# q8888620002/Group-Attribution-for-Diffusion-Models

Hardware: AMD Instinct MI355X
Metric: shapley_coalitions_per_hour (higher is better)
Workload: dtype f32; 1 GPU; CIFAR-20 DDPM sFT coalition (BASELINE configs[1]): gd_steps=1000 @B=128 + 10240 samples x 100 DDIM steps @B=32 (32 batches fused/launch), UNet2DModel widths [128, 256, 256, 256] 35.75M params fp32; step = 1/1000 coalition = 1 train step + 1 sampler step @B=1024, enqueued on 3 HIP streams (the train step belongs to a later coalition: independent work); coalitions_in_flight=3

## Files before the change

group-attribution-for-diffusion-models_amd/csrc/gemm_f32.hip:

```cpp
#include "gad_common.h"
#include "gemm_dev.h"

using namespace gadk;

namespace gadk {
void launch_wino4_fused(const DevArgs& w, int bm, hipStream_t st);
}

namespace {

template <int ROWS, int VEC>
struct LoadKCDense : KCSlots<ROWS> {
  using S = KCSlots<ROWS>;
  const float* base;
  long roff[S::NS];
  unsigned rowmask;
  int kend, k;
  bool kok;
  __device__ void init(const float* b, int ld, int row0, int nrows, int kend_) {
    base = b;
    kend = kend_;
    rowmask = 0;
#pragma unroll
    for (int i = 0; i < S::NS; ++i) {
// ... 2067 lines not shown

static int pick_vec(const gad_gemm_args* a) {
  int vec = 4;
  const int am = a->a_mode, bmode = a->b_mode;
  if (am == GAD_A_KC && (a->K % 4 != 0 || a->lda % 4 != 0)) vec = 1;
  if (am == GAD_A_MC && (a->M % 4 != 0 || a->lda % 4 != 0)) vec = 1;
  if (bmode == GAD_B_KC && (a->K % 4 != 0 || a->ldb % 4 != 0)) vec = 1;
  if (bmode == GAD_B_MC && (a->N % 4 != 0 || a->ldb % 4 != 0)) vec = 1;
  if ((am == GAD_A_CONV || am == GAD_A_CONVT || bmode == GAD_B_CONV) && (a->g.C % 4 != 0 || a->g.ldx % 4 != 0)) vec = 1;
  if (a->batch > 1 && (a->strideA0 % 4 != 0 || a->strideA1 % 4 != 0 || a->strideB0 % 4 != 0 || a->strideB1 % 4 != 0)) vec = 1;
  return vec;
}

enum : int32_t {
  HINT_128 = 1,
  HINT_64 = 2,
  HINT_128x64 = 3,
  HINT_WGRAD_96 = 4, HINT_WGRAD_64 = 5, HINT_WGRAD_32 = 6,
  HINT_WINO2 = 7,
  HINT_WINO4 = 8,
  HINT_WINO4_FUSED32 = 9,
  HINT_WINO4_THREE = 10,
  HINT_WINO4_FUSED64 = 11,
  HINT_SPLIT_M = 1000,
};

struct Plan {
  int bm, bn, tiles_m, tiles_n, splitk, ktiles_per_split;
  long nblocks;
};

static bool dense_128x64_ok(const gad_gemm_args* a) {
  const bool dense = (a->a_mode == GAD_A_KC || a->a_mode == GAD_A_MC) && (a->b_mode == GAD_B_KC || a->b_mode == GAD_B_MC) &&
                     !(a->a_mode == GAD_A_MC && a->b_mode == GAD_B_KC);
  return dense && !a->A2 && pick_vec(a) == 4 && !(a->operand_precision == 1);
}
static Plan make_plan(const gad_gemm_args* a) {
  const long batch = a->batch > 0 ? a->batch : 1;
  const int kt = (int)gad_ceil_div(a->K, BK) > 0 ? (int)gad_ceil_div(a->K, BK) : 1;
  static const int sks[] = {1, 2, 3, 4, 6, 8, 12, 16, 24, 32, 48, 64, 96, 128};
  double best = 1e30;
  Plan pl{};
  for (int bm = 128; bm >= 64; bm -= 64) {
    if (a->tile_hint == HINT_128 && bm != 128) continue;
    if (a->tile_hint == HINT_64 && bm != 64) continue;
    const bool bf = a->operand_precision == 1 && pick_vec(a) == 4;
// ... 350 lines not shown
  PatchPlan pp;
  if (use_patch_conv_f32(a, &pp)) {
    t_direct = (double)gad_ceil_div(pp.blocks, 512) * pp.chunks_per_split * 9.0 * (128.0 * pp.bn * 64.0) / 0.264e12;
    if (pp.splitk > 1) t_direct += 4e-6 + (double)a->M * a->N * 4.0 * (pp.splitk + 1) / 3.0e12;
  } else {
    t_direct = 2.0 * a->M * (double)a->N * a->K / 110e12;
  }
  const double tw = t2 < t4 ? t2 : t4;
  if (!(tw < 0.9 * t_direct)) return false;
  *wp = t2 < t4 ? p2 : p4;
  return true;
}

struct WinoWgradPlan {
  long T;
  int64_t wy_bytes, v_bytes, du_bytes, bytes;
};
static bool use_wino_wgrad(const gad_gemm_args* a, WinoWgradPlan* wq) {
  const gad_conv_geom& g = a->g;
  if (!(a->flags & GAD_GEMM_WINO_WGRAD) || (a->flags & (GAD_GEMM_NO_WINO | GAD_GEMM_NO_PATCH | GAD_GEMM_INTERNAL_WINO4))) return false;
  if (a->operand_precision != 0 || a->a_mode != GAD_A_MC || a->b_mode != GAD_B_CONV || a->A2 || a->A_k2 || a->batch > 1) return false;
  if (!same_3x3(g) || (g.Ho & 3) || (g.Wo & 3)) return false;
  if (g.C % 4 != 0 || g.ldx % 4 != 0 || a->M % 4 != 0 || a->lda % 4 != 0 || a->N != 9 * g.C || a->ldc % 4 != 0) return false;
  if ((a->tile_hint != 0 && a->tile_hint != HINT_WINO4) || a->splitk_hint > 0 || a->K % (g.Ho * g.Wo) != 0) return false;
  if (a->alpha != 1.f || a->bias || a->rowadd || a->residual) return false;
  if (!(gad_aligned16(a->A) && gad_aligned16(a->B) && gad_aligned16(a->C))) return false;
  wq->T = (long)a->K / 16;
  wq->wy_bytes = (int64_t)36 * wq->T * a->M * 4;
  wq->v_bytes = (int64_t)36 * wq->T * g.C * 4;
  wq->du_bytes = (int64_t)36 * a->M * g.C * 4;
  wq->bytes = wq->wy_bytes + wq->v_bytes + wq->du_bytes;
  if (a->tile_hint == HINT_WINO4) return true;
  const double dy_bytes = 4.0 * a->K * a->M, x_bytes = 4.0 * (double)(a->K / (g.Ho * g.Wo)) * g.H * g.W * g.C;
  const double t_w = (dy_bytes + x_bytes + (double)wq->wy_bytes + (double)wq->v_bytes) / 4.9e12 + 36.0 * wq->T * a->M * (double)g.C * 2.0 / 100e12 +
                     3.0 * (double)wq->du_bytes / 3.0e12 + 30e-6;
  const double t_direct = 2.0 * a->K * (double)a->M * a->N / 115e12;
  return t_w < 0.9 * t_direct;
}


static gad_gemm_args products36(const gad_gemm_args* a, const float* A, const float* B, float* C, int am, int bm, int M, int N, int K) {
  gad_gemm_args sub = *a;
  sub.A = A; sub.B = B; sub.C = C;
  sub.a_mode = am; sub.b_mode = bm;
  sub.M = M; sub.N = N; sub.K = K;
  sub.lda = am == GAD_A_MC ? M : K; sub.ldb = bm == GAD_B_MC ? N : K; sub.ldc = N;
  sub.batch = 36; sub.batch_inner = 1;
  sub.strideA0 = (int64_t)M * K; sub.strideB0 = (int64_t)N * K; sub.strideC0 = (int64_t)M * N;
  sub.strideA1 = sub.strideB1 = sub.strideC1 = 0;
  sub.tile_hint = 0; sub.splitk_hint = 0;
  sub.flags = GAD_GEMM_INTERNAL_WINO4;
  sub.B_wino = nullptr; sub.B_wino4 = nullptr; sub.wino_ws = nullptr; sub.wino_ws_bytes = 0;
  sub.A2 = nullptr;
  return sub;
}
// ... 257 lines not shown
  GAD_CHECK(a->wino_ws && a->wino_ws_bytes >= wq.bytes && gad_aligned16(a->wino_ws),
            "gad_gemm: Winograd weight-gradient workspace too small or misaligned (%lld < %lld)", (long long)a->wino_ws_bytes, (long long)wq.bytes);
  float* Wy = (float*)a->wino_ws;
  float* V = Wy + wq.wy_bytes / 4;
  float* dU = V + wq.v_bytes / 4;
  const bool have_v = (a->flags & GAD_GEMM_WINO_SKIP_INPUT) && a->B_wino4 != nullptr;
  if (have_v) {
    GAD_CHECK(gad_aligned16(a->B_wino4), "gad_gemm: the kept Winograd input image (B_wino4 of a weight-gradient launch) must be 16-byte aligned");
    V = const_cast<float*>(a->B_wino4);
  }
  WinoIn wy;
  wy.x = a->A; wy.V = Wy;
  wy.H = g.Ho; wy.W = g.Wo; wy.C = a->M; wy.ldx = a->lda; wy.up = 0;
  wy.TH = g.Ho / 4; wy.TW = g.Wo / 4; wy.T = wq.T;
  WinoIn wi;
  wi.x = a->B; wi.V = V;
  wi.H = g.H; wi.W = g.W; wi.C = g.C; wi.ldx = g.ldx; wi.up = g.upsample ? 1 : 0;
  wi.TH = wy.TH; wi.TW = wy.TW; wi.T = wq.T;
  const long iy = wq.T * (a->M / 4), ix = wq.T * (g.C / 4);
  GAD_CHECK(gad_ceil_div(iy, 256) < (1L << 31) && gad_ceil_div(ix, 256) < (1L << 31), "gad_gemm: Winograd transform grid too large");
  hipLaunchKernelGGL(wino4_dy_kernel, dim3((unsigned)gad_ceil_div(iy, 256)), dim3(256), 0, st, wy);
  if (!have_v) hipLaunchKernelGGL(wino4_input_kernel, dim3((unsigned)gad_ceil_div(ix, 256)), dim3(256), 0, st, wi);
  GAD_LAUNCH_CHECK("gad_gemm(winograd wgrad transforms)");
  const gad_gemm_args sub = wino_wgrad_products_args(a, wq, Wy, V, dU);
  if (const int rc = gad_gemm(&sub, stream)) return rc;
  const long items = (long)a->M * (g.C / 4);
  hipLaunchKernelGGL(wino4_dw_kernel, dim3((unsigned)gad_ceil_div(items, 256)), dim3(256), 0, st, dU, a->C, a->M, g.C, a->ldc);
  GAD_LAUNCH_CHECK("gad_gemm(winograd wgrad output transform)");
  return 0;
}

static int launch_wino(const Route& r, const DevArgs& d, void* stream) {
  const gad_gemm_args* a = &r.a;
  const WinoPlan& wp = r.wp;
  const gad_conv_geom& g = a->g;
  hipStream_t st = (hipStream_t)stream;
  GAD_CHECK(a->wino_ws && a->wino_ws_bytes >= wp.bytes && gad_aligned16(a->wino_ws) && gad_aligned16(wp.f == 2 ? a->B_wino : a->B_wino4),
            "gad_gemm: Winograd workspace too small or misaligned (%lld < %lld)", (long long)a->wino_ws_bytes, (long long)wp.bytes);
  WinoIn wi;
  wi.x = a->A; wi.V = (float*)a->wino_ws;
  wi.H = g.H; wi.W = g.W; wi.C = g.C; wi.ldx = g.ldx; wi.up = g.upsample ? 1 : 0;
  wi.TH = g.Ho / wp.f; wi.TW = g.Wo / wp.f; wi.T = wp.T;
  const long items = wp.T * (g.C / 4);
  GAD_CHECK(gad_ceil_div(items, 256) < (1L << 31), "gad_gemm: Winograd input transform grid too large");
  const bool only_input = (a->flags & GAD_GEMM_WINO_ONLY_INPUT) != 0, skip_input = (a->flags & GAD_GEMM_WINO_SKIP_INPUT) != 0;
  auto products = [&](const float* U) {
    DevArgs w = d;
    w.A = wi.V; w.B = U;
// ... 260 lines not shown
```

group-attribution-for-diffusion-models_amd/gad/_capi.py:

```python
import ctypes as C
import os

_HERE = os.path.dirname(os.path.abspath(__file__))
LIB_PATH = os.path.join(_HERE, "libgad_hip.so")


class GadError(RuntimeError):
    pass


class ConvGeom(C.Structure):
    _fields_ = [("H", C.c_int32), ("W", C.c_int32), ("C", C.c_int32), ("ldx", C.c_int32),
                ("Ho", C.c_int32), ("Wo", C.c_int32), ("KH", C.c_int32), ("KW", C.c_int32),
                ("stride", C.c_int32), ("pad_t", C.c_int32), ("pad_l", C.c_int32), ("upsample", C.c_int32)]


class GemmArgs(C.Structure):
    _fields_ = [("A", C.c_void_p), ("B", C.c_void_p), ("C", C.c_void_p),
                ("a_mode", C.c_int32), ("b_mode", C.c_int32),
                ("M", C.c_int32), ("N", C.c_int32), ("K", C.c_int32),
                ("lda", C.c_int32), ("ldb", C.c_int32), ("ldc", C.c_int32),
                ("batch", C.c_int32), ("batch_inner", C.c_int32),
                ("strideA0", C.c_int64), ("strideA1", C.c_int64), ("strideB0", C.c_int64),
                ("strideB1", C.c_int64), ("strideC0", C.c_int64), ("strideC1", C.c_int64),
# ... 49 lines not shown
                ("tile_hint", C.c_int32), ("splitk_hint", C.c_int32)]


class AdamArgs(C.Structure):
    _fields_ = [("p", C.c_void_p), ("g", C.c_void_p), ("m", C.c_void_p), ("v", C.c_void_p), ("ema", C.c_void_p),
                ("n", C.c_int64), ("sumsq", C.c_void_p), ("max_norm", C.c_float),
                ("lr", C.c_float), ("beta1", C.c_float), ("beta2", C.c_float), ("eps", C.c_float),
                ("weight_decay", C.c_float), ("adamw", C.c_int32), ("step", C.c_int32), ("ema_decay", C.c_float)]


class JLArgs(C.Structure):
    _fields_ = [("A", C.c_void_p), ("lda", C.c_int64), ("G", C.c_int32), ("P", C.c_int64), ("p0", C.c_int64),
                ("d", C.c_int32), ("seed", C.c_uint32), ("model_id", C.c_uint32), ("type", C.c_int32),
                ("accumulate", C.c_int32), ("out", C.c_void_p), ("workspace", C.c_void_p), ("workspace_bytes", C.c_int64)]


class HGemmSegArgs(C.Structure):
    _fields_ = [("A", C.c_void_p), ("B", C.c_void_p), ("C", C.c_void_p), ("ws", C.c_void_p), ("ws_bytes", C.c_int64),
                ("c_seg_stride", C.c_int64), ("M", C.c_int32), ("N", C.c_int32), ("L", C.c_int32), ("S", C.c_int32),
                ("lda", C.c_int32), ("ldb", C.c_int32), ("ldc", C.c_int32), ("alpha", C.c_float), ("accumulate", C.c_int32),
                ("splitk_hint", C.c_int32)]


JL_NORMAL, JL_RADEMACHER = 0, 1
POOL_MAX, POOL_AVG, POOL_AVG_VALID = 0, 1, 2
GELU_ERF, GELU_QUICK = 0, 1
SIM_X_F32, SIM_X_U8 = 0, 1

GEMM_NO_PATCH, GEMM_TAP_MAJOR_K, GEMM_SCALAR_EPILOGUE, GEMM_GENERAL_LOADERS, GN_TWO_PASS = 1, 2, 4, 8, 1
GEMM_NO_WINO = 16
GEMM_WINO_WGRAD = 32
GEMM_WINO_ONLY_INPUT, GEMM_WINO_SKIP_INPUT = 64, 128
A_KC, A_MC, A_CONV, A_CONVT = 0, 1, 2, 3
B_KC, B_MC, B_WDGRAD, B_CONV = 0, 1, 2, 3

_vp, _i32, _i64, _f32, _f64 = C.c_void_p, C.c_int32, C.c_int64, C.c_float, C.c_double

SIGNATURES = {
    "gad_version": (C.c_int, []),
    "gad_last_error": (C.c_char_p, []),
    "gad_gemm_workspace_bytes": (_i64, [C.POINTER(GemmArgs)]),
    "gad_gemm": (C.c_int, [C.POINTER(GemmArgs), _vp]),
    "gad_gemm_uses_bf16": (C.c_int, [C.POINTER(GemmArgs)]),
    "gad_gemm_kernel_id": (C.c_int, [C.POINTER(GemmArgs)]),
    "gad_gemm_wino_bytes": (_i64, [C.POINTER(GemmArgs)]),
    "gad_wino_weights": (C.c_int, [_vp, _vp, _vp, _i64, _vp]),
    "gad_wino4_weights": (C.c_int, [_vp, _vp, _vp, _i64, _vp]),
    "gad_groupnorm_one_pass": (C.c_int, [C.POINTER(GroupNormArgs)]),
    "gad_gemm_plan": (C.c_int, [C.POINTER(GemmArgs), C.POINTER(_i32), C.POINTER(_i32), C.POINTER(_i32)]),
    "gad_groupnorm_workspace_bytes": (_i64, [C.POINTER(GroupNormArgs)]),
    "gad_groupnorm_silu_fwd": (C.c_int, [C.POINTER(GroupNormArgs), _vp]),
    "gad_groupnorm_silu_bwd": (C.c_int, [C.POINTER(GroupNormArgs), _vp]),
    "gad_groupnorm_wino4_ok": (C.c_int, [C.POINTER(GroupNormArgs), C.c_int32]),
    "gad_groupnorm_silu_wino4": (C.c_int, [C.POINTER(GroupNormArgs), _vp, C.c_int32, _vp]),
    "gad_attention_supported": (C.c_int, [_i32]),
    "gad_attention_uses_bf16": (C.c_int, [C.POINTER(AttentionArgs), _i32]),
    "gad_attention_bwd_workspace_bytes": (_i64, [C.POINTER(AttentionArgs)]),
    "gad_attention_fwd": (C.c_int, [C.POINTER(AttentionArgs), _vp]),
    "gad_attention_bwd": (C.c_int, [C.POINTER(AttentionArgs), _vp]),
    "gad_attention_d512_supported": (C.c_int, [_i32]),
    "gad_attention_fwd_d512": (C.c_int, [C.POINTER(AttentionArgs), _vp]),
    "gad_attention_causal_supported": (C.c_int, [_i32, _i32]),
    "gad_attention_causal_fwd": (C.c_int, [C.POINTER(AttentionArgs), _vp]),
    "gad_softmax_fwd": (C.c_int, [_vp, _vp, _i64, _i32, _f32, _vp]),
    "gad_softmax_bwd": (C.c_int, [_vp, _vp, _vp, _i64, _i32, _f32, _vp]),
    "gad_layernorm_workspace_bytes": (_i64, [_i64, _i32]),
    "gad_layernorm_fwd": (C.c_int, [_vp, _vp, _vp, _vp, _vp, _vp, _i64, _i32, _f32, _vp]),
    "gad_layernorm_bwd": (C.c_int, [_vp, _vp, _vp, _vp, _vp, _vp, _vp, _vp, _i64, _i32, _vp, _i64, _vp]),
    "gad_geglu_fwd": (C.c_int, [_vp, _vp, _i64, _i32, _vp]),
    "gad_geglu_bwd": (C.c_int, [_vp, _vp, _vp, _i64, _i32, _vp]),
# ... 91 lines not shown
```

group-attribution-for-diffusion-models_amd/gad/ops.py:

```python
from __future__ import annotations

import ctypes as C
import math
from typing import Optional

import torch

from . import _capi
from ._capi import (A_CONV, A_CONVT, A_KC, A_MC, B_CONV, B_KC, B_MC, B_WDGRAD, AdamArgs, ConvGeom, GemmArgs,
                    GroupNormArgs, check)
from .shadows import (WEIGHT_EPOCH, Shadow, cached, in_flat_buffer as _in_flat_buffer, weight_key, written,
                      written_everywhere)

_WS = {}
WS_BYTES = 1 << 30


def _stream():
    return C.c_void_p(torch.cuda.current_stream().cuda_stream)


_raw_stream = getattr(torch._C, "_cuda_getCurrentRawStream", None)


# ... 201 lines not shown
                a.B_wino4 = wino_v.data_ptr()
                a.flags |= _capi.GEMM_WINO_SKIP_INPUT
        else:
            a.flags &= ~_capi.GEMM_WINO_WGRAD
    if wino_input is not None:
        if lib.gad_gemm_kernel_id(C.byref(a)) != 6 or not a.wino_ws:
            return False
        wino_input(V)
        a.flags |= _capi.GEMM_WINO_SKIP_INPUT
    if ROUTE_STATS is not None and (a.B_wino4 or a.flags & _capi.GEMM_WINO_WGRAD):
        key = (lib.gad_gemm_kernel_id(C.byref(a)), M, N, K, bool(a.flags & _capi.GEMM_WINO_SKIP_INPUT), torch.is_grad_enabled())
        ROUTE_STATS[key] = ROUTE_STATS.get(key, 0) + 1
    if SCRATCH_ALLOC is not None:
        need = lib.gad_gemm_workspace_bytes(C.byref(a))
        ws = _scratch("ws", need, A.device) if need else None
        a.ws, a.ws_bytes = (ws.data_ptr() if need else None), need
    if PROFILER is not None:
        PROFILER.gemm(lib, a, batch)
        return True
    check(lib.gad_gemm(C.byref(a), _stream()), "gad_gemm")
    return True


class GemmProfiler:
    NAMES = {(A_CONV, B_KC): "conv_fwd", (A_CONVT, B_WDGRAD): "conv_dgrad", (A_MC, B_CONV): "conv_wgrad",
             (A_KC, B_KC): "gemm_nt", (A_KC, B_MC): "gemm_nn", (A_MC, B_MC): "gemm_tn"}

    def __init__(self):
        self.records = []

    def gemm(self, lib, a, batch):
        tile, sk, vec = C.c_int32(), C.c_int32(), C.c_int32()
        check(lib.gad_gemm_plan(C.byref(a), C.byref(tile), C.byref(sk), C.byref(vec)), "gad_gemm_plan")
        kid = lib.gad_gemm_kernel_id(C.byref(a))
        s, e, mid = torch.cuda.Event(enable_timing=True), torch.cuda.Event(enable_timing=True), None
        s.record()
        if kid in (5, 6) and not (a.flags & _capi.GEMM_WINO_SKIP_INPUT):
            flags = a.flags
            mid = torch.cuda.Event(enable_timing=True)
            a.flags = flags | _capi.GEMM_WINO_ONLY_INPUT
            check(lib.gad_gemm(C.byref(a), _stream()), "gad_gemm")
            mid.record()
            a.flags = flags | _capi.GEMM_WINO_SKIP_INPUT
            check(lib.gad_gemm(C.byref(a), _stream()), "gad_gemm")
            a.flags = flags
        else:
            check(lib.gad_gemm(C.byref(a), _stream()), "gad_gemm")
        e.record()
        name = self.NAMES.get((a.a_mode, a.b_mode), "gemm") + ("", "_bf16", f"_patch_w{a.g.Wo}", f"_patch_bf16_w{a.g.Wo}", f"_fewout_valu_w{a.g.Wo}", "_wino", "_wino4", "_wino4")[kid]
        key = (name, tile.value, sk.value, vec.value)
        g = a.g
        if a.a_mode in (A_CONV, A_CONVT):
            a_elems = (a.M // max(1, g.Ho * g.Wo)) * g.H * g.W * g.C
        else:
            a_elems = a.M * a.K
        b_elems = (a.K // max(1, g.Ho * g.Wo)) * g.H * g.W * g.C if a.b_mode == B_CONV else a.N * a.K
        extra = a.M * a.N if a.residual else 0
        nbytes = 4.0 * max(1, batch) * (a_elems + b_elems + a.M * a.N + extra)
        flops = 2.0 * a.M * a.N * a.K * max(1, batch)
        executed = flops * ({5: 16.0 / 36.0, 6: 0.25, 7: 0.25}.get(kid, 1.0))
        stage = None
        if kid in (5, 6):
            npos, tpx = (16, 4) if kid == 5 else (36, 16)
            v_bytes = 4.0 * npos * (a.M // tpx) * g.C
            stage = (mid, 4.0 * a_elems + v_bytes if mid is not None else 0.0, v_bytes + 4.0 * (b_elems * npos / 9.0 + a.M * a.N + extra))
        self.records.append((key, flops, nbytes, s, e, executed, stage))

    def hgemm(self, lib, a, tn=False):
        s, e = torch.cuda.Event(enable_timing=True), torch.cuda.Event(enable_timing=True)
        if tn:
            s.record()
            check(lib.gad_hgemm_tn(C.byref(a), _stream()), "gad_hgemm_tn")
            e.record()
            nbytes = 2.0 * a.K * (a.M + a.N) + 4.0 * a.M * a.N
            flops = 2.0 * a.M * a.N * a.K
            self.records.append((("hgemm_tn_wgrad", 128, 0, 8), flops, nbytes, s, e, flops, None))
            return
        tile, sk = C.c_int32(), C.c_int32()
        check(lib.gad_hgemm_plan(C.byref(a), C.byref(tile), C.byref(sk)), "gad_hgemm_plan")
        s.record()
        check(lib.gad_hgemm(C.byref(a), _stream()), "gad_hgemm")
        e.record()
        if a.conv:
            name = f"hconv{a.KH}x{a.KW}" + ("_s2dgrad" if a.conv == 2 else "_s2" if a.stride == 2 else "_up" if a.upsample else "")
            a_elems = (a.M // max(1, a.Ho * a.Wo)) * a.H * a.W * a.Cin
        else:
            name = "hgemm_wgrad" if a.out_f32 else "hgemm_lora" if a.A2 else "hgemm"
            a_elems = a.M * a.K
        nbytes = 2.0 * (a_elems + a.N * a.K + (a.M * a.N if a.residual else 0)) + (4.0 if a.out_f32 else 2.0) * a.M * a.N
        flops = 2.0 * a.M * a.N * a.K
# ... 238 lines not shown
        return dxe
    g = ConvGeom(Ho, Wo, Cout, Cout, He, We, KH, KW, stride, pad[0], pad[2], 0)
    gemm_raw(dy, wk, dxe, A_CONVT, B_WDGRAD, Bn * He * We, Cin, KH * KW * Cout, 0, 0, Cin, geom=g,
             tile_hint=tile_hint, splitk_hint=splitk_hint)
    return _upsample2x_bwd(dxe, x_shape) if upsample else dxe


def _upsample2x_bwd(dxe, x_shape):
    Bn, H, W, Cin = x_shape
    dx = torch.empty((Bn, H, W, Cin), device=dxe.device, dtype=torch.float32)
    check(_capi.load().gad_upsample2x_bwd(dxe.data_ptr(), dx.data_ptr(), Bn, H, W, Cin, _stream()), "gad_upsample2x_bwd")
    return dx


def conv2d_wgrad_raw(dy, x, w_like, stride=1, pad=(1, 1, 1, 1), upsample=False, tile_hint=0, splitk_hint=0, out=None, wino_v=None):
    _req(dy, "conv dy")
    _req(x, "conv x")
    Bn, H, W, Cin = x.shape
    Cout, _, KH, KW = w_like.shape
    _, Ho, Wo, _ = dy.shape
    dwk = _out((Cout, KH, KW, Cin), dy.device) if out is None else weight_krsc(out)
    if (KH == 1 and KW == 1 and stride == 1 and tuple(pad) == (0, 0, 0, 0) and not upsample and Cin % 4 == 0 and Cout % 4 == 0
            and not KERNEL_FLAGS["gemm"] & _capi.GEMM_GENERAL_LOADERS):
        gemm_raw(dy, x, dwk, A_MC, B_MC, Cout, Cin, Bn * H * W, Cout, Cin, Cin, tile_hint=tile_hint, splitk_hint=splitk_hint)
        return dwk.permute(0, 3, 1, 2)
    g = ConvGeom(H, W, Cin, Cin, Ho, Wo, KH, KW, stride, pad[0], pad[2], int(upsample))
    wino = (KH == 3 and KW == 3 and stride == 1 and tuple(pad) == (1, 1, 1, 1) and tile_hint in (0, 8) and splitk_hint == 0
            and Ho % 4 == 0 and Wo % 4 == 0 and OPERAND_PRECISION[0] == 0 and not KERNEL_FLAGS.get("no_wino4")
            and not KERNEL_FLAGS["gemm"] & (_capi.GEMM_NO_WINO | _capi.GEMM_NO_PATCH | _capi.GEMM_SCALAR_EPILOGUE | _capi.GEMM_TAP_MAJOR_K
                                            | _capi.GEMM_GENERAL_LOADERS))
    gemm_raw(dy, x, dwk, A_MC, B_CONV, Cout, KH * KW * Cin, Bn * Ho * Wo, Cout, 0, KH * KW * Cin, geom=g,
             tile_hint=tile_hint, splitk_hint=splitk_hint, wino_wgrad=wino, wino_v=wino_v)
    return dwk.permute(0, 3, 1, 2)


def colsum_raw(dy2d: torch.Tensor, segments=1, out=None):
    lib = _capi.load()
    ws = workspace(dy2d.device)
    rows, N = dy2d.shape
    if out is None:
        out = torch.empty((segments, N), device=dy2d.device, dtype=torch.float32)
    check(lib.gad_colsum(dy2d.data_ptr(), out.data_ptr(), segments, rows // segments, N, ws.data_ptr(), ws.numel(),
                         _stream()), "gad_colsum")
    return out


def linear_fwd_raw(x2d, w, bias=None, residual=None, alpha=1.0, force_f32=False):
    M, K = x2d.shape
    N = w.shape[0]
    y = _out((M, N), x2d.device)
# ... 146 lines not shown

def layernorm_fwd_raw(x, gamma, beta, eps):
    C_ = x.shape[-1]
    rows = x.numel() // C_
    y = torch.empty_like(x)
    stats = torch.empty((2, rows), device=x.device, dtype=torch.float32)
    check(_capi.load().gad_layernorm_fwd(x.data_ptr(), y.data_ptr(), gamma.data_ptr(), beta.data_ptr(), stats[0].data_ptr(),
                                         stats[1].data_ptr(), rows, C_, eps, _stream()), "gad_layernorm_fwd")
    return y, stats[0], stats[1]


def linear_dgrad_raw(dy2d, w):
    M, N = dy2d.shape
    K = w.shape[1]
    dx = _out((M, K), dy2d.device)
    gemm_raw(dy2d, w, dx, A_KC, B_MC, M, K, N, N, K, K)
    return dx


def linear_wgrad_raw(dy2d, x2d, out=None):
    M, N = dy2d.shape
    K = x2d.shape[1]
    dw = _out((N, K), dy2d.device) if out is None else out
    gemm_raw(dy2d, x2d, dw, A_MC, B_MC, N, K, M, N, K, K)
    return dw


def _param_grad(param, compute):
    v, first = _sink(param)
    if v is None:
        return compute(None)
    if first:
        compute(v)
    else:
        v.add_(compute(None))
    return None


def _conv_backward(ctx, dy, x, x_shape, w, stride, pad, upsample, has, need):
    dy = dy.contiguous()
    dx = None
    if need[0]:
        if dgrad_as_forward(w, stride, pad):
            dx = conv2d_fwd_raw(dy, rotated_weight(w), None)
            if upsample:
                dx = _upsample2x_bwd(dx, x_shape)
        else:
# ... 829 lines not shown
```

include/gad.h:

```cpp
#ifndef GAD_H
#define GAD_H
#include <stdint.h>
#ifdef __cplusplus
extern "C" {
#endif

int gad_version(void);
const char* gad_last_error(void);

enum gad_a_mode {
  GAD_A_KC = 0,
  GAD_A_MC = 1,
  GAD_A_CONV = 2,
  GAD_A_CONVT = 3
};
enum gad_b_mode {
  GAD_B_KC = 0,
  GAD_B_MC = 1,
  GAD_B_WDGRAD = 2,
  GAD_B_CONV = 3
};

typedef struct gad_conv_geom {
  int32_t H, W, C;
// ... 37 lines not shown
  void* wino_ws;
  int64_t wino_ws_bytes;
  const float* B_wino4;
} gad_gemm_args;
enum gad_gemm_flags {
  GAD_GEMM_NO_WINO = 16,
  GAD_GEMM_WINO_WGRAD = 32,
  GAD_GEMM_NO_PATCH = 1,
  GAD_GEMM_TAP_MAJOR_K = 2,
  GAD_GEMM_SCALAR_EPILOGUE = 4,
  GAD_GEMM_GENERAL_LOADERS = 8,
  GAD_GEMM_WINO_ONLY_INPUT = 64,
  GAD_GEMM_WINO_SKIP_INPUT = 128
};

int64_t gad_gemm_workspace_bytes(const gad_gemm_args* a);
int gad_gemm_plan(const gad_gemm_args* a, int32_t* tile, int32_t* splitk, int32_t* vec);
int gad_gemm(const gad_gemm_args* a, void* stream);
int gad_gemm_uses_bf16(const gad_gemm_args* a);
int gad_gemm_kernel_id(const gad_gemm_args* a);
int64_t gad_gemm_wino_bytes(const gad_gemm_args* a);
int gad_wino_weights(const float* src, float* dst, const int64_t* table, int64_t n_tiles, void* stream);
int gad_wino4_weights(const float* src, float* dst, const int64_t* table, int64_t n_tiles, void* stream);

typedef struct gad_groupnorm_args {
  const float* x;
  float* y;
  const float* gamma;
  const float* beta;
  float* mean;
  float* rstd;
  const float* dy;
  float* dgamma;
  float* dbeta;
  int32_t B, HW, C, G;
  float eps;
  int32_t silu;
  void* ws;
  int64_t ws_bytes;
  const float* x2;
  int32_t C1;
  int32_t flags;
  const float* dx_add;
} gad_groupnorm_args;
enum gad_groupnorm_flags { GAD_GN_TWO_PASS = 1 };

// ... 225 lines not shown
```

Baseline: 45.81 coalitions/hour.

## Add dedicated TN split-K GEMM kernel for weight gradients and Winograd products

```diff
diff --git a/group-attribution-for-diffusion-models_amd/csrc/gemm_f32.hip b/group-attribution-for-diffusion-models_amd/csrc/gemm_f32.hip
--- a/group-attribution-for-diffusion-models_amd/csrc/gemm_f32.hip
+++ b/group-attribution-for-diffusion-models_amd/csrc/gemm_f32.hip
@@ -2113,6 +2113,7 @@
   HINT_WINO4_FUSED32 = 9,
   HINT_WINO4_THREE = 10,
   HINT_WINO4_FUSED64 = 11,
+  HINT_WINO4_TN = 12,
   HINT_SPLIT_M = 1000,
 };
 
@@ -2509,7 +2510,7 @@
   if (a->operand_precision != 0 || a->a_mode != GAD_A_MC || a->b_mode != GAD_B_CONV || a->A2 || a->A_k2 || a->batch > 1) return false;
   if (!same_3x3(g) || (g.Ho & 3) || (g.Wo & 3)) return false;
   if (g.C % 4 != 0 || g.ldx % 4 != 0 || a->M % 4 != 0 || a->lda % 4 != 0 || a->N != 9 * g.C || a->ldc % 4 != 0) return false;
-  if ((a->tile_hint != 0 && a->tile_hint != HINT_WINO4) || a->splitk_hint > 0 || a->K % (g.Ho * g.Wo) != 0) return false;
+  if ((a->tile_hint != 0 && a->tile_hint != HINT_WINO4 && a->tile_hint != HINT_WINO4_TN) || a->splitk_hint > 0 || a->K % (g.Ho * g.Wo) != 0) return false;
   if (a->alpha != 1.f || a->bias || a->rowadd || a->residual) return false;
   if (!(gad_aligned16(a->A) && gad_aligned16(a->B) && gad_aligned16(a->C))) return false;
   wq->T = (long)a->K / 16;
@@ -2517,7 +2518,7 @@
   wq->v_bytes = (int64_t)36 * wq->T * g.C * 4;
   wq->du_bytes = (int64_t)36 * a->M * g.C * 4;
   wq->bytes = wq->wy_bytes + wq->v_bytes + wq->du_bytes;
-  if (a->tile_hint == HINT_WINO4) return true;
+  if (a->tile_hint == HINT_WINO4 || a->tile_hint == HINT_WINO4_TN) return true;
   const double dy_bytes = 4.0 * a->K * a->M, x_bytes = 4.0 * (double)(a->K / (g.Ho * g.Wo)) * g.H * g.W * g.C;
   const double t_w = (dy_bytes + x_bytes + (double)wq->wy_bytes + (double)wq->v_bytes) / 4.9e12 + 36.0 * wq->T * a->M * (double)g.C * 2.0 / 100e12 +
                      3.0 * (double)wq->du_bytes / 3.0e12 + 30e-6;
@@ -2821,8 +2822,28 @@
   hipLaunchKernelGGL(wino4_dy_kernel, dim3((unsigned)gad_ceil_div(iy, 256)), dim3(256), 0, st, wy);
   if (!have_v) hipLaunchKernelGGL(wino4_input_kernel, dim3((unsigned)gad_ceil_div(ix, 256)), dim3(256), 0, st, wi);
   GAD_LAUNCH_CHECK("gad_gemm(winograd wgrad transforms)");
-  const gad_gemm_args sub = wino_wgrad_products_args(a, wq, Wy, V, dU);
-  if (const int rc = gad_gemm(&sub, stream)) return rc;
+  const bool tn_wanted = a->tile_hint == HINT_WINO4_TN || (a->M <= 128 && g.C <= 128 && (a->M > 64 || g.C > 64) && wq.T >= 4096);
+  gad_gemm_tn_args tn;
+  memset(&tn, 0, sizeof(tn));
+  tn.A = Wy; tn.B = V; tn.C = dU;
+  tn.M = a->M; tn.N = g.C; tn.K = (int32_t)wq.T;
+  tn.lda = a->M; tn.ldb = g.C; tn.ldc = g.C;
+  tn.batch = 36;
+  tn.strideA = wq.T * a->M; tn.strideB = wq.T * g.C; tn.strideC = (int64_t)a->M * g.C;
+  const int64_t tn_need = tn_wanted ? gad_gemm_tn_workspace_bytes(&tn) : -1;
+  int32_t tn_tile = 0, tn_splits = 0, tn_slab = 0;
+  if (tn_wanted && tn_need >= 0 && gad_gemm_tn_plan(&tn, &tn_tile, &tn_splits, &tn_slab) == 0) {
+    if (tn_splits == 1) tn_tile = 1;
+    else if (have_v && tn_need <= wq.v_bytes) { tn.ws = Wy + wq.wy_bytes / 4; tn.ws_bytes = wq.v_bytes; }
+    else if (!have_v && a->ws && gad_aligned16(a->ws) && tn_need <= a->ws_bytes && tn_need <= workspace_bytes(r)) { tn.ws = a->ws; tn.ws_bytes = a->ws_bytes; }
+    else tn_tile = 0;
+  } else tn_tile = 0;
+  if (tn_tile) {
+    if (const int rc = gad_gemm_tn(&tn, stream)) return rc;
+  } else {
+    const gad_gemm_args sub = wino_wgrad_products_args(a, wq, Wy, V, dU);
+    if (const int rc = gad_gemm(&sub, stream)) return rc;
+  }
   const long items = (long)a->M * (g.C / 4);
   hipLaunchKernelGGL(wino4_dw_kernel, dim3((unsigned)gad_ceil_div(items, 256)), dim3(256), 0, st, dU, a->C, a->M, g.C, a->ldc);
   GAD_LAUNCH_CHECK("gad_gemm(winograd wgrad output transform)");
diff --git a/group-attribution-for-diffusion-models_amd/csrc/gemm_tn_f32.hip b/group-attribution-for-diffusion-models_amd/csrc/gemm_tn_f32.hip
--- /dev/null
+++ b/group-attribution-for-diffusion-models_amd/csrc/gemm_tn_f32.hip
@@ -0,0 +1,306 @@
+#include "gemm_dev.h"
+
+using namespace gadk;
+
+namespace {
+
+template <int N>
+__device__ __forceinline__ void wait_vm() {
+  static_assert(N >= 0 && N < 64, "vmcnt is 6 bits on gfx9");
+  __builtin_amdgcn_s_waitcnt((N & 15) | ((N >> 4) << 14) | 0x0F70);
+}
+template <int N>
+__device__ __forceinline__ void barrier_vm() {
+  static_assert(N >= 0 && N < 64, "vmcnt is 6 bits on gfx9");
+  asm volatile("s_waitcnt vmcnt(%0)\n\ts_barrier" ::"n"(N) : "memory");
+}
+
+struct TnDev {
+  const float* A;
+  const float* B;
+  float* C;
+  float* ws;
+  int M, N, K, lda, ldb, ldc, batch;
+  long sA, sB, sC;
+  int tiles_m, tiles_n, splits, slab;
+};
+
+template <int ROWS>
+struct TnRows : MCSlots<ROWS> {
+  using S = MCSlots<ROWS>;
+  const float* ptr;
+  long step;
+  long ld;
+  int k, kend;
+  __device__ void init(const float* b, int ld_, int col0, int ncols, int kbeg, int kend_) {
+    int c0 = col0 + S::rq4();
+    c0 = c0 < ncols ? c0 : ncols - 4;
+    ld = ld_;
+    step = (long)BK * ld_;
+    k = kbeg + S::krow(0);
+    kend = kend_;
+    ptr = b + (long)k * ld_ + c0;
+  }
+  __device__ __forceinline__ const float* src(int i) const {
+    return sel_src(ptr, (long)(S::KSTEP * i) * ld, k + S::KSTEP * i < kend);
+  }
+  __device__ __forceinline__ void advance() {
+    ptr += step;
+    k += BK;
+  }
+};
+
+__device__ __forceinline__ void store_tile(const f32x16& acc, float* scratch, float* C, int ldc, int m0, int n, int M, bool n_ok,
+                                           int h, int l31) {
+  const int lane = l31 + 32 * h, rr = lane >> 3, c4 = (lane & 7) * 4;
+#pragma unroll
+  for (int e = 0; e < 16; ++e) scratch[((e & 3) + 8 * (e >> 2) + 4 * h) * EPI_LD + l31] = acc[e];
+#pragma unroll
+  for (int q = 0; q < 4; ++q) {
+    const int r = rr + 8 * q;
+    const f32x4 v = *reinterpret_cast<const f32x4*>(scratch + r * EPI_LD + c4);
+    const int m = m0 + r;
+    if (m < M && n_ok) *reinterpret_cast<f32x4*>(C + (long)m * ldc + n) = v;
+  }
+}
+
+template <int BM, int BN, int NST>
+__global__ __launch_bounds__(NTHREADS, BM == 128 ? 1 : 2) void gemm_tn_f32_kernel(const TnDev p) {
+  constexpr int TM = BM / 64, TN = BN / 64, D = NST - 1, NACC = 4;
+  constexpr int A_TILE = BK * BM, STAGE = BK * (BM + BN);
+  using AL = TnRows<BM>;
+  using BL = TnRows<BN>;
+  constexpr int NDMA = AL::NS + BL::NS;
+  static_assert(NDMA <= 16, "one DMA per piece of a step");
+  static_assert(NDMA * (D - 1) < 64, "vmcnt");
+  static_assert(NST >= 3 && NST * STAGE >= 4 * EPI_WAVE, "the epilogue scratch lives in the ring");
+  __shared__ __attribute__((aligned(16))) float lds[NST * STAGE];
+
+  const int t = xcd_remap(blockIdx.x, gridDim.x);
+  const int tiles = p.tiles_m * p.tiles_n;
+  const int zs = t / tiles, rem = t - zs * tiles;
+  const int tile_m = rem / p.tiles_n, tile_n = rem - tile_m * p.tiles_n;
+  const int z = zs / p.splits, split = zs - z * p.splits;
+  const int row0 = tile_m * BM, col0 = tile_n * BN;
+  const int kbeg = split * p.slab;
+  const int kend = min(p.K, kbeg + p.slab);
+  const int nkt = (kend - kbeg + BK - 1) / BK;
+
+  AL al;
+  BL bl;
+  al.init(p.A + z * p.sA, p.lda, row0, p.M, kbeg, kend);
+  bl.init(p.B + z * p.sB, p.ldb, col0, p.N, kbeg, kend);
+
+  const int tid = threadIdx.x, wave = tid >> 6, lane = tid & 63;
+  const int wm = wave >> 1, wn = wave & 1, h = lane >> 5, l31 = lane & 31;
+
+  f32x16 acc[NACC][TM][TN];
+#pragma unroll
+  for (int c = 0; c < NACC; ++c)
+#pragma unroll
+    for (int i = 0; i < TM; ++i)
+#pragma unroll
+      for (int j = 0; j < TN; ++j)
+#pragma unroll
+        for (int e = 0; e < 16; ++e) acc[c][i][j][e] = 0.f;
+
+  auto issue = [&](int d, float* stage) {
+    if (d < AL::NS) glds16(al.src(d), AL::dma_dst(stage, d));
+    else glds16(bl.src(d - AL::NS), BL::dma_dst(stage + A_TILE, d - AL::NS));
+  };
+#pragma unroll
+  for (int s = 0; s < D; ++s) {
+#pragma unroll
+    for (int d = 0; d < NDMA; ++d) issue(d, lds + s * STAGE);
+    al.advance();
+    bl.advance();
+  }
+  barrier_vm<NDMA * (D - 1)>();
+
+  int cs = 0;
+  auto step = [&](f32x16 (&acc)[TM][TN]) {
+    const float* la = lds + cs * STAGE;
+    const float* lb = la + A_TILE;
+    float* pf = lds + (cs == 0 ? NST - 1 : cs - 1) * STAGE;
+    f32x4 fa[2][TM], fb[2][TN];
+#pragma unroll
+    for (int i = 0; i < TM; ++i) fa[0][i] = read_frag<false, BM>(la, wm * (BM / 2) + i * 32 + l31, 0, h);
+#pragma unroll
+    for (int j = 0; j < TN; ++j) fb[0][j] = read_frag<false, BN>(lb, wn * (BN / 2) + j * 32 + l31, 0, h);
+#pragma unroll
+    for (int g = 0; g < 4; ++g) {
+#pragma unroll
+      for (int s = 0; s < 4; ++s) {
+#pragma unroll
+        for (int i = 0; i < TM; ++i)
+#pragma unroll
+          for (int j = 0; j < TN; ++j)
+            acc[i][j] = __builtin_amdgcn_mfma_f32_32x32x2f32(fa[g & 1][i][s], fb[g & 1][j][s], acc[i][j], 0, 0, 0);
+        if (g * 4 + s < NDMA) issue(g * 4 + s, pf);
+        if (s == 1 && g < 3) {
+#pragma unroll
+          for (int i = 0; i < TM; ++i) fa[(g + 1) & 1][i] = read_frag<false, BM>(la, wm * (BM / 2) + i * 32 + l31, g + 1, h);
+#pragma unroll
+          for (int j = 0; j < TN; ++j) fb[(g + 1) & 1][j] = read_frag<false, BN>(lb, wn * (BN / 2) + j * 32 + l31, g + 1, h);
+        }
+#pragma unroll
+        for (int q = 0; q < TM * TN; ++q) {
+          __builtin_amdgcn_sched_group_barrier(0x008, 1, 0);
+          __builtin_amdgcn_sched_group_barrier(0x002, 7, 0);
+        }
+        __builtin_amdgcn_sched_barrier(0);
+      }
+    }
+    al.advance();
+    bl.advance();
+    cs = cs + 1 == NST ? 0 : cs + 1;
+    barrier_vm<NDMA * (D - 1)>();
+  };
+  static_assert(NACC == 4, "the loop below deals the steps to four sets");
+  for (int kt = 0; kt < nkt; kt += NACC) {
+    step(acc[0]);
+    if (kt + 1 < nkt) step(acc[1]);
+    if (kt + 2 < nkt) step(acc[2]);
+    if (kt + 3 < nkt) step(acc[3]);
+  }
+#pragma unroll
+  for (int i = 0; i < TM; ++i)
+#pragma unroll
+    for (int j = 0; j < TN; ++j) acc[0][i][j] = (acc[0][i][j] + acc[1][i][j]) + (acc[2][i][j] + acc[3][i][j]);
+  wait_vm<0>();
+  __syncthreads();
+
+  const bool direct = p.splits == 1;
+  float* C = direct ? p.C + z * p.sC : p.ws + ((long)split * p.batch + z) * p.M * p.N;
+  const int ldc = direct ? p.ldc : p.N;
+  float* scratch = lds + wave * EPI_WAVE;
+  const int c4 = (lane & 7) * 4;
+#pragma unroll
+  for (int j = 0; j < TN; ++j) {
+    const int n = col0 + wn * (BN / 2) + j * 32 + c4;
+#pragma unroll
+    for (int i = 0; i < TM; ++i) store_tile(acc[0][i][j], scratch, C, ldc, row0 + wm * (BM / 2) + i * 32, n, p.M, n < p.N, h, l31);
+  }
+}
+
+__global__ __launch_bounds__(256) void gemm_tn_reduce_kernel(const TnDev p) {
+  const long mn = (long)p.M * p.N, total4 = (long)p.batch * mn / 4;
+  for (long i4 = (long)blockIdx.x * blockDim.x + threadIdx.x; i4 < total4; i4 += (long)gridDim.x * blockDim.x) {
+    const long idx = i4 * 4;
+    const int z = (int)(idx / mn);
+    const long r = idx - (long)z * mn;
+    const int m = (int)(r / p.N), n = (int)(r - (long)m * p.N);
+    const float* w = p.ws + idx;
+    f32x4 v = zero4();
+    for (int s = 0; s < p.splits; ++s) v += ldg4(w + (long)s * p.batch * mn);
+    *reinterpret_cast<f32x4*>(p.C + z * p.sC + (long)m * p.ldc + n) = v;
+  }
+}
+
+constexpr int TN_MIN_K = 8192;
+constexpr long TN_MIN_MN = 128L * 256, TN_MAX_MN = 256L * 256;
+constexpr int TN_MIN_STEPS = 16;
+
+struct TnPlan {
+  int tile, tiles_m, tiles_n, splits, slab;
+  long blocks;
+};
+
+static int tn_batch(const gad_gemm_tn_args* a) { return a->batch > 0 ? a->batch : 1; }
+
+static const char* tn_contract(const gad_gemm_tn_args* a) {
+  if (!a || !a->A || !a->B || !a->C) return "null operand";
+  if (a->M < 4 || a->N < 4 || a->K < 1) return "empty problem";
+  if (a->M % 4 != 0 || a->N % 4 != 0) return "M and N must be multiples of 4";
+  if (a->lda % 4 != 0 || a->ldb % 4 != 0 || a->ldc % 4 != 0) return "lda, ldb and ldc must be multiples of 4";
+  if (a->lda < a->M || a->ldb < a->N || a->ldc < a->N) return "lda < M, ldb < N or ldc < N";
+  if (!gad_aligned16(a->A) || !gad_aligned16(a->B) || !gad_aligned16(a->C)) return "operands must be 16-byte aligned";
+  if (a->batch > 1 && (a->strideA % 4 != 0 || a->strideB % 4 != 0 || a->strideC % 4 != 0)) return "batch strides must be multiples of 4";
+  if (a->batch > 1 && (a->strideA < 0 || a->strideB < 0 || a->strideC < (int64_t)(a->M - 1) * a->ldc + a->N)) return "batch strides: outputs would overlap";
+  if (a->K > (1 << 30) || (int64_t)a->K * (a->lda > a->ldb ? a->lda : a->ldb) >= (1LL << 40)) return "operand too large";
+  if (a->tile_hint != 0 && a->tile_hint != 64 && a->tile_hint != 128) return "tile_hint must be 0, 64 or 128";
+  if (a->splitk_hint < 0) return "splitk_hint < 0";
+  return nullptr;
+}
+
+static TnPlan tn_plan(const gad_gemm_tn_args* a) {
+  TnPlan pl;
+  const long batch = tn_batch(a);
+  const bool one_128 = batch >= 8 && a->M <= 128 && a->N <= 128 && (a->M > 64 || a->N > 64);
+  pl.tile = a->tile_hint ? a->tile_hint : (one_128 ? 128 : 64);
+  pl.tiles_m = (int)gad_ceil_div(a->M, pl.tile);
+  pl.tiles_n = (int)gad_ceil_div(a->N, pl.tile);
+  const long tiles = (long)pl.tiles_m * pl.tiles_n * batch;
+  const long slots = 256L * (pl.tile == 128 ? 1 : 2);
+  const long nkt = gad_ceil_div(a->K, BK);
+  long want;
+  if (a->splitk_hint > 0) want = a->splitk_hint;
+  else {
+    want = slots / tiles > 0 ? slots / tiles : 1;
+    const long most = nkt / TN_MIN_STEPS > 0 ? nkt / TN_MIN_STEPS : 1;
+    want = want < most ? want : most;
+  }
+  want = want < nkt ? want : nkt;
+  const long per = gad_ceil_div(nkt, want);
+  pl.splits = (int)gad_ceil_div(nkt, per);
+  pl.slab = (int)(per * BK);
+  pl.blocks = tiles * pl.splits;
+  return pl;
+}
+
+static int64_t tn_bytes(const gad_gemm_tn_args* a, const TnPlan& pl) {
+  return (int64_t)pl.splits * tn_batch(a) * a->M * a->N * (int64_t)sizeof(float);
+}
+
+}
+
+extern "C" int gad_gemm_tn_ok(const gad_gemm_tn_args* a) {
+  return tn_contract(a) == nullptr && a->batch <= 1 && a->K >= TN_MIN_K && (long)a->M * a->N >= TN_MIN_MN && (long)a->M * a->N <= TN_MAX_MN ? 1 : 0;
+}
+
+extern "C" int gad_gemm_tn_plan(const gad_gemm_tn_args* a, int32_t* tile, int32_t* splits, int32_t* slab_tokens) {
+  GAD_CHECK(tile && splits && slab_tokens, "gad_gemm_tn_plan: null pointer");
+  const char* why = tn_contract(a);
+  GAD_CHECK(!why, "gad_gemm_tn_plan: %s", why);
+  const TnPlan pl = tn_plan(a);
+  *tile = pl.tile;
+  *splits = pl.splits;
+  *slab_tokens = pl.slab;
+  return 0;
+}
+
+extern "C" int64_t gad_gemm_tn_workspace_bytes(const gad_gemm_tn_args* a) {
+  const char* why = tn_contract(a);
+  if (why) {
+    gad_set_error("gad_gemm_tn_workspace_bytes: %s", why);
+    return -1;
+  }
+  return tn_bytes(a, tn_plan(a));
+}
+
+extern "C" int gad_gemm_tn(const gad_gemm_tn_args* a, void* stream) {
+  const char* why = tn_contract(a);
+  GAD_CHECK(!why, "gad_gemm_tn: %s", why);
+  const TnPlan pl = tn_plan(a);
+  GAD_CHECK(pl.blocks < (1L << 31), "gad_gemm_tn: grid too large");
+  if (pl.splits > 1)
+    GAD_CHECK(a->ws && gad_aligned16(a->ws) && a->ws_bytes >= tn_bytes(a, pl), "gad_gemm_tn: split workspace too small or misaligned (%lld < %lld)",
+              (long long)a->ws_bytes, (long long)tn_bytes(a, pl));
+  TnDev d;
+  d.A = a->A; d.B = a->B; d.C = a->C; d.ws = (float*)a->ws;
+  d.M = a->M; d.N = a->N; d.K = a->K; d.lda = a->lda; d.ldb = a->ldb; d.ldc = a->ldc; d.batch = tn_batch(a);
+  d.sA = a->batch > 1 ? a->strideA : 0; d.sB = a->batch > 1 ? a->strideB : 0; d.sC = a->batch > 1 ? a->strideC : 0;
+  d.tiles_m = pl.tiles_m; d.tiles_n = pl.tiles_n; d.splits = pl.splits; d.slab = pl.slab;
+  hipStream_t st = (hipStream_t)stream;
+  const dim3 grid((unsigned)pl.blocks), block(NTHREADS);
+  if (pl.tile == 128) hipLaunchKernelGGL((gemm_tn_f32_kernel<128, 128, 3>), grid, block, 0, st, d);
+  else hipLaunchKernelGGL((gemm_tn_f32_kernel<64, 64, 3>), grid, block, 0, st, d);
+  GAD_LAUNCH_CHECK("gemm_tn_f32_kernel");
+  if (pl.splits > 1) {
+    const long items = (long)d.batch * d.M * d.N / 4;
+    const long blocks = gad_ceil_div(items, 256) < 2048 ? gad_ceil_div(items, 256) : 2048;
+    hipLaunchKernelGGL(gemm_tn_reduce_kernel, dim3((unsigned)blocks), dim3(256), 0, st, d);
+    GAD_LAUNCH_CHECK("gemm_tn_reduce_kernel");
+  }
+  return 0;
+}
diff --git a/group-attribution-for-diffusion-models_amd/gad/_capi.py b/group-attribution-for-diffusion-models_amd/gad/_capi.py
--- a/group-attribution-for-diffusion-models_amd/gad/_capi.py
+++ b/group-attribution-for-diffusion-models_amd/gad/_capi.py
@@ -95,6 +95,15 @@
                 ("splitk_hint", C.c_int32)]
 
 
+class GemmTnArgs(C.Structure):
+    _fields_ = [("A", C.c_void_p), ("B", C.c_void_p), ("C", C.c_void_p),
+                ("M", C.c_int32), ("N", C.c_int32), ("K", C.c_int32),
+                ("lda", C.c_int32), ("ldb", C.c_int32), ("ldc", C.c_int32), ("batch", C.c_int32),
+                ("strideA", C.c_int64), ("strideB", C.c_int64), ("strideC", C.c_int64),
+                ("ws", C.c_void_p), ("ws_bytes", C.c_int64),
+                ("tile_hint", C.c_int32), ("splitk_hint", C.c_int32)]
+
+
 JL_NORMAL, JL_RADEMACHER = 0, 1
 POOL_MAX, POOL_AVG, POOL_AVG_VALID = 0, 1, 2
 GELU_ERF, GELU_QUICK = 0, 1
@@ -119,6 +128,10 @@
     "gad_gemm_wino_bytes": (_i64, [C.POINTER(GemmArgs)]),
     "gad_wino_weights": (C.c_int, [_vp, _vp, _vp, _i64, _vp]),
     "gad_wino4_weights": (C.c_int, [_vp, _vp, _vp, _i64, _vp]),
+    "gad_gemm_tn_ok": (C.c_int, [C.POINTER(GemmTnArgs)]),
+    "gad_gemm_tn_plan": (C.c_int, [C.POINTER(GemmTnArgs), C.POINTER(_i32), C.POINTER(_i32), C.POINTER(_i32)]),
+    "gad_gemm_tn_workspace_bytes": (_i64, [C.POINTER(GemmTnArgs)]),
+    "gad_gemm_tn": (C.c_int, [C.POINTER(GemmTnArgs), _vp]),
     "gad_groupnorm_one_pass": (C.c_int, [C.POINTER(GroupNormArgs)]),
     "gad_gemm_plan": (C.c_int, [C.POINTER(GemmArgs), C.POINTER(_i32), C.POINTER(_i32), C.POINTER(_i32)]),
     "gad_groupnorm_workspace_bytes": (_i64, [C.POINTER(GroupNormArgs)]),
diff --git a/group-attribution-for-diffusion-models_amd/gad/ops.py b/group-attribution-for-diffusion-models_amd/gad/ops.py
--- a/group-attribution-for-diffusion-models_amd/gad/ops.py
+++ b/group-attribution-for-diffusion-models_amd/gad/ops.py
@@ -247,6 +247,29 @@
     return True
 
 
+def gemm_tn_raw(A, B, Cout, M, N, K, lda, ldb, ldc, batch=1, strides=(0, 0, 0), tile_hint=0, splitk_hint=0, force=False):
+    if OPERAND_PRECISION[0] or KERNEL_FLAGS["gemm"]:
+        return False
+    lib = _capi.load()
+    a = _capi.GemmTnArgs()
+    a.A, a.B, a.C = A.data_ptr(), B.data_ptr(), Cout.data_ptr()
+    a.M, a.N, a.K, a.lda, a.ldb, a.ldc, a.batch = M, N, K, lda, ldb, ldc, batch
+    a.strideA, a.strideB, a.strideC = strides
+    a.tile_hint, a.splitk_hint = tile_hint, splitk_hint
+    if not force and not lib.gad_gemm_tn_ok(C.byref(a)):
+        return False
+    need = lib.gad_gemm_tn_workspace_bytes(C.byref(a))
+    if need < 0:
+        raise _capi.GadError(f"gad_gemm_tn: {lib.gad_last_error().decode()}")
+    ws = _scratch("ws", need, A.device) if SCRATCH_ALLOC is not None else workspace(A.device)
+    a.ws, a.ws_bytes = ws.data_ptr(), ws.numel()
+    if PROFILER is not None:
+        PROFILER.gemm_tn(lib, a)
+        return True
+    check(lib.gad_gemm_tn(C.byref(a), _stream()), "gad_gemm_tn")
+    return True
+
+
 class GemmProfiler:
     NAMES = {(A_CONV, B_KC): "conv_fwd", (A_CONVT, B_WDGRAD): "conv_dgrad", (A_MC, B_CONV): "conv_wgrad",
              (A_KC, B_KC): "gemm_nt", (A_KC, B_MC): "gemm_nn", (A_MC, B_MC): "gemm_tn"}
@@ -291,6 +314,17 @@
             stage = (mid, 4.0 * a_elems + v_bytes if mid is not None else 0.0, v_bytes + 4.0 * (b_elems * npos / 9.0 + a.M * a.N + extra))
         self.records.append((key, flops, nbytes, s, e, executed, stage))
 
+    def gemm_tn(self, lib, a):
+        tile, sk, slab = C.c_int32(), C.c_int32(), C.c_int32()
+        check(lib.gad_gemm_tn_plan(C.byref(a), C.byref(tile), C.byref(sk), C.byref(slab)), "gad_gemm_tn_plan")
+        s, e = torch.cuda.Event(enable_timing=True), torch.cuda.Event(enable_timing=True)
+        s.record()
+        check(lib.gad_gemm_tn(C.byref(a), _stream()), "gad_gemm_tn")
+        e.record()
+        batch = max(1, a.batch)
+        flops = 2.0 * a.M * a.N * a.K * batch
+        self.records.append((("gemm_tn", tile.value, sk.value, 4), flops, 4.0 * batch * (a.K * (a.M + a.N) + a.M * a.N), s, e, flops, None))
+
     def hgemm(self, lib, a, tn=False):
         s, e = torch.cuda.Event(enable_timing=True), torch.cuda.Event(enable_timing=True)
         if tn:
@@ -575,10 +609,11 @@
     dwk = _out((Cout, KH, KW, Cin), dy.device) if out is None else weight_krsc(out)
     if (KH == 1 and KW == 1 and stride == 1 and tuple(pad) == (0, 0, 0, 0) and not upsample and Cin % 4 == 0 and Cout % 4 == 0
             and not KERNEL_FLAGS["gemm"] & _capi.GEMM_GENERAL_LOADERS):
-        gemm_raw(dy, x, dwk, A_MC, B_MC, Cout, Cin, Bn * H * W, Cout, Cin, Cin, tile_hint=tile_hint, splitk_hint=splitk_hint)
+        if tile_hint or splitk_hint or not gemm_tn_raw(dy, x, dwk, Cout, Cin, Bn * H * W, Cout, Cin, Cin):
+            gemm_raw(dy, x, dwk, A_MC, B_MC, Cout, Cin, Bn * H * W, Cout, Cin, Cin, tile_hint=tile_hint, splitk_hint=splitk_hint)
         return dwk.permute(0, 3, 1, 2)
     g = ConvGeom(H, W, Cin, Cin, Ho, Wo, KH, KW, stride, pad[0], pad[2], int(upsample))
-    wino = (KH == 3 and KW == 3 and stride == 1 and tuple(pad) == (1, 1, 1, 1) and tile_hint in (0, 8) and splitk_hint == 0
+    wino = (KH == 3 and KW == 3 and stride == 1 and tuple(pad) == (1, 1, 1, 1) and tile_hint in (0, 8, 12) and splitk_hint == 0
             and Ho % 4 == 0 and Wo % 4 == 0 and OPERAND_PRECISION[0] == 0 and not KERNEL_FLAGS.get("no_wino4")
             and not KERNEL_FLAGS["gemm"] & (_capi.GEMM_NO_WINO | _capi.GEMM_NO_PATCH | _capi.GEMM_SCALAR_EPILOGUE | _capi.GEMM_TAP_MAJOR_K
                                             | _capi.GEMM_GENERAL_LOADERS))
@@ -771,7 +806,8 @@
     M, N = dy2d.shape
     K = x2d.shape[1]
     dw = _out((N, K), dy2d.device) if out is None else out
-    gemm_raw(dy2d, x2d, dw, A_MC, B_MC, N, K, M, N, K, K)
+    if not gemm_tn_raw(dy2d, x2d, dw, N, K, M, N, K, K):
+        gemm_raw(dy2d, x2d, dw, A_MC, B_MC, N, K, M, N, K, K)
     return dw
 
 
diff --git a/include/gad.h b/include/gad.h
--- a/include/gad.h
+++ b/include/gad.h
@@ -83,6 +83,24 @@
 int64_t gad_gemm_wino_bytes(const gad_gemm_args* a);
 int gad_wino_weights(const float* src, float* dst, const int64_t* table, int64_t n_tiles, void* stream);
 int gad_wino4_weights(const float* src, float* dst, const int64_t* table, int64_t n_tiles, void* stream);
+
+typedef struct gad_gemm_tn_args {
+  const float* A;
+  const float* B;
+  float* C;
+  int32_t M, N, K;
+  int32_t lda, ldb, ldc;
+  int32_t batch;
+  int64_t strideA, strideB, strideC;
+  void* ws;
+  int64_t ws_bytes;
+  int32_t tile_hint;
+  int32_t splitk_hint;
+} gad_gemm_tn_args;
+int gad_gemm_tn_ok(const gad_gemm_tn_args* a);
+int gad_gemm_tn_plan(const gad_gemm_tn_args* a, int32_t* tile, int32_t* splits, int32_t* slab_tokens);
+int64_t gad_gemm_tn_workspace_bytes(const gad_gemm_tn_args* a);
+int gad_gemm_tn(const gad_gemm_tn_args* a, void* stream);
 
 typedef struct gad_groupnorm_args {
   const float* x;
```

Result: no change. 45.75 coalitions/hour (-0.1%).
